# titisda/graph-python

Hardware: AMD Instinct MI355X
Metric: GTEPS (masked mxv/vxm level-BFS, R-MAT s22) (higher is better)
Workload: dtype bool; 1 GPU; level-BFS q<!v.S,replace> = q any.pair A (GxB_ANY_PAIR_BOOL; GrB_vxm, GrB_mxv on A^T shards for N>1), R-MAT scale 22, edge factor 16, 16 roots; n=4194304, nnz=65243197, parallelism=single GPU

## Files before the change

### graph-python_amd/csrc/gb_context.cpp

```cpp
#include <algorithm>
#include <chrono>
#include <cstdio>
#include <cstdio>
#include <cstdlib>
#include <atomic>
#include <map>
#include <mutex>
#include <unordered_map>
#include <vector>

#include <cstring>
#include <dlfcn.h>

#include "gb_internal.h"

namespace {
bool g_init = false;
int g_device = 0;
hipStream_t g_own_stream = nullptr;
hipStream_t g_user_stream = nullptr;
bool g_user_stream_set = false;
std::mutex g_knob_mu;
std::map<std::string, int64_t> g_knobs;
std::atomic<bool> g_any_knob{false};
// ... 314 lines not shown
    g_live[p] = cls;
    return p;
}

void gb_free(void *p) {
    if (!p) return;
    std::lock_guard<std::mutex> lk(g_mem_mu);
    auto it = g_live.find(p);
    if (it == g_live.end()) {
        (void)hipFreeAsync(p, gb_stream());
        return;
    }
    size_t cls = it->second;
    g_live.erase(it);
    if (cls > kCacheLimit) {
        (void)hipFreeAsync(p, gb_stream());
        return;
    }
    while (g_cached_bytes + cls > kCacheLimit && !g_lru.empty()) evict_oldest_locked();
    const uint64_t seq = ++g_free_seq;
    g_cache[cls].push_back(gb_cached{p, seq});
    g_lru.emplace(seq, std::make_pair(p, cls));
    g_cached_bytes += cls;
}

void gb_memset(void *p, int v, size_t bytes) {
    if (bytes) GB_HIP(hipMemsetAsync(p, v, bytes, gb_stream()));
}
void gb_copy_d2d(void *dst, const void *src, size_t bytes) {
    if (bytes) GB_HIP(hipMemcpyAsync(dst, src, bytes, hipMemcpyDeviceToDevice, gb_stream()));
}
void gb_copy_h2d(void *dst, const void *src, size_t bytes) {
    if (bytes) GB_HIP(hipMemcpyAsync(dst, src, bytes, hipMemcpyHostToDevice, gb_stream()));
}
void gb_copy_d2h(void *dst, const void *src, size_t bytes) {
    if (bytes && bytes <= kPinned) {
        std::lock_guard<std::mutex> lk(g_pin_mu);
        if (!g_pinned) GB_HIP(hipHostMalloc(&g_pinned, kPinned, hipHostMallocDefault));
        GB_HIP(hipMemcpyAsync(g_pinned, src, bytes, hipMemcpyDeviceToHost, gb_stream()));
        gb_sync();
        memcpy(dst, g_pinned, bytes);
        return;
    }
    if (bytes) GB_HIP(hipMemcpyAsync(dst, src, bytes, hipMemcpyDeviceToHost, gb_stream()));
    gb_sync();
}
int64_t gb_read_i64(const int64_t *dptr) {
    int64_t v = 0;
    gb_copy_d2h(&v, dptr, sizeof(v));
    return v;
}

int64_t gb_iso_ts_dump();

static const char *k_type_names[] = {"BOOL", "INT8", "UINT8", "INT16", "UINT16", "INT32",
                                     "UINT32", "INT64", "UINT64", "FP32", "FP64"};
static const size_t k_type_sizes[] = {1, 1, 1, 2, 2, 4, 4, 8, 8, 4, 8};
const char *gb_type_name(int code) { return k_type_names[code]; }
size_t gb_type_size(int code) { return k_type_sizes[code]; }
GrB_Type gb_type_of(int code) {
    switch (code) {
    case GBAMD_T_BOOL: return GrB_BOOL;
    case GBAMD_T_INT8: return GrB_INT8;
    case GBAMD_T_UINT8: return GrB_UINT8;
    case GBAMD_T_INT16: return GrB_INT16;
    case GBAMD_T_UINT16: return GrB_UINT16;
    case GBAMD_T_INT32: return GrB_INT32;
    case GBAMD_T_UINT32: return GrB_UINT32;
    case GBAMD_T_INT64: return GrB_INT64;
    case GBAMD_T_UINT64: return GrB_UINT64;
    case GBAMD_T_FP32: return GrB_FP32;
    default: return GrB_FP64;
    }
}

gb_desc gb_read_desc(const GrB_Descriptor d) {
    gb_desc r;
    if (!d) return r;
    GB_REQUIRE(d->magic == GB_MAGIC, GrB_UNINITIALIZED_OBJECT, "invalid descriptor");
    r.replace = d->outp == GrB_REPLACE;
    r.comp = (d->mask & GrB_COMP) != 0;
    r.structure = (d->mask & GrB_STRUCTURE) != 0;
    r.tran0 = d->inp0 == GrB_TRAN;
    r.tran1 = d->inp1 == GrB_TRAN;
    return r;
}

extern "C" {

static int32_t g_mode = GrB_NONBLOCKING;

GrB_Info GrB_init(GrB_Mode mode) {
    return gb_api(nullptr, [&] {
        GB_REQUIRE(!g_init, GrB_INVALID_VALUE, "GrB_init called twice");
        GB_REQUIRE(mode == GrB_BLOCKING || mode == GrB_NONBLOCKING, GrB_INVALID_VALUE, "invalid mode");
        gb_do_init();
        g_mode = mode;
    });
}

GrB_Info GxB_Global_Option_get_INT32(GxB_Option_Field field, int32_t *value) {
    if (!value) return GrB_NULL_POINTER;
    if (field != GxB_MODE) return GrB_INVALID_VALUE;
    *value = g_mode;
    return GrB_SUCCESS;
}

GrB_Info GrB_finalize(void) {
    return gb_api(nullptr, [&] {
        if (!g_init) return;
        GB_HIP(hipDeviceSynchronize());
    });
}

GrB_Info GrB_getVersion(unsigned int *version, unsigned int *subversion) {
    if (!version || !subversion) return GrB_NULL_POINTER;
    *version = GRB_VERSION;
    *subversion = GRB_SUBVERSION;
    return GrB_SUCCESS;
}

GrB_Info GxB_Context_set_stream(void *hip_stream) {
    return gb_api(nullptr, [&] {
        gb_require_init();
        GB_HIP(hipStreamSynchronize(gb_stream()));
        g_user_stream = (hipStream_t)hip_stream;
        g_user_stream_set = hip_stream != nullptr;
    });
}

GrB_Info GxB_Context_get_stream(void **hip_stream) {
    if (!hip_stream) return GrB_NULL_POINTER;
    return gb_api(nullptr, [&] { *hip_stream = (void *)gb_stream(); });
}

GrB_Info GxB_Context_set_device(int device) {
    if (g_init) return GrB_INVALID_VALUE;
    g_device = device;
    return GrB_SUCCESS;
}

GrB_Info GxB_Global_set_int(const char *key, int64_t value) {
    if (!key) return GrB_NULL_POINTER;
    std::lock_guard<std::mutex> lk(g_knob_mu);
    g_knobs[key] = value;
    if (!strcmp(key, "grid_cap")) g_grid_cap.store(value > 0 ? value : 0, std::memory_order_relaxed);
    g_any_knob.store(true, std::memory_order_release);
    return GrB_SUCCESS;
}

GrB_Info GxB_Global_get_int(const char *key, int64_t *value) {
    if (!key || !value) return GrB_NULL_POINTER;
    if (gb_deferred_stat(key, value)) return GrB_SUCCESS;
    if (!strcmp(key, "stat_spmv_host_push")) {
        *value = g_stat_host_push.load(std::memory_order_relaxed);
        return GrB_SUCCESS;
    }
    if (!strcmp(key, "stat_nvals_copy")) {
        *value = g_stat_nvals_copy.load(std::memory_order_relaxed);
        return GrB_SUCCESS;
    }
    if (!strcmp(key, "iso_ts_dump")) {
        return gb_api(nullptr, [&] { *value = gb_iso_ts_dump(); });
    }
    {
        bool mine = false;
        const GrB_Info info = gb_api(nullptr, [&] { mine = gb_sort_stat(key, value) || gb_selectk_stat(key, value); });
        if (mine || info != GrB_SUCCESS) return info;
    }
    if (!strncmp(key, "stat_", 5)) {
        const GrB_Info info = gb_api(nullptr, [&] { gb_union_stat_refresh(key); });
        if (info != GrB_SUCCESS) return info;
        if (!gb_stat_get(key + 5, value)) *value = 0;
        return GrB_SUCCESS;
    }
    *value = gb_knob(key);
    return GrB_SUCCESS;
}

GrB_Info GxB_builtin_lookup(void **handle, int *kind, const char *name) {
    if (!handle || !kind || !name) return GrB_NULL_POINTER;
    static std::map<std::string, const GB_builtin_entry *> *idx = nullptr;
    static std::mutex mu;
    {
        std::lock_guard<std::mutex> lk(mu);
        if (!idx) {
            idx = new std::map<std::string, const GB_builtin_entry *>();
            for (const GB_builtin_entry *e = GB_builtin_registry; e->name; e++) (*idx)[e->name] = e;
        }
    }
    auto it = idx->find(name);
    if (it == idx->end()) return GrB_INVALID_VALUE;
    *handle = it->second->obj;
    *kind = it->second->kind;
    return GrB_SUCCESS;
}

GrB_Info GxB_name(const char **name, const void *obj) {
    if (!name || !obj) return GrB_NULL_POINTER;
    for (const GB_builtin_entry *e = GB_builtin_registry; e->name; e++) {
        if (e->obj == obj) {
            *name = e->name;
            return GrB_SUCCESS;
        }
    }
    return GrB_INVALID_VALUE;
// ... 88 lines not shown
```

### graph-python_amd/csrc/gb_internal.h

```cpp
#pragma once
#include <atomic>
#include <utility>
#include <hip/hip_runtime.h>

#include <cstdint>
#include <cstring>
#include <stdexcept>
#include <string>
#include <vector>

#include "../../include/gbamd_codes.h"
#include "gb_state.h"
#include "../../include/graphblas_amd.h"

#define GB_MAGIC 0x6d614d424731ULL
#define GB_FREED 0x646565724642ULL

struct GB_Type_opaque {
    uint64_t magic;
    int code;
    size_t size;
    const char *name;
};
struct GB_BinaryOp_opaque {
// ... 231 lines not shown
struct gb_scratch {
    void *ptrs[32];
    int n = 0;
    template <class T>
    T *get(size_t count) {
        T *p = gb_malloc_n<T>(count ? count : 1);
        ptrs[n++] = p;
        return p;
    }
    ~gb_scratch() {
        for (int i = 0; i < n; i++) gb_free(ptrs[i]);
    }
};

GB_Obj *gb_obj_check(const void *p, bool allow_null = false);
GB_Obj *gb_obj_check_raw(const void *p, bool allow_null = false);
void gb_cw_to_csr(GB_Obj *A);
void gb_cw_release(GB_Obj *A);
void gb_cw_materialize(GB_Obj *A);
GB_Obj *gb_new_object(int kind, GrB_Type type, int64_t nrows, int64_t ncols);
extern "C" void gb_vec_recount(GB_Obj *v);
void gb_obj_free_storage(GB_Obj *A);
void gb_drop_transpose(GB_Obj *A);
int64_t gb_nvals(GB_Obj *A);
inline int64_t gb_words(int64_t n) { return (n + 63) >> 6; }
inline bool gb_is_bitmap(const GB_Obj *A) { return A->kind != GB_KIND_MATRIX; }

void gb_cast_array(void *dst, int dst_code, const void *src, int src_code, int64_t n);

struct gb_csr_view {
    int64_t nrows = 0, ncols = 0, nvals = 0;
    const int64_t *rowptr = nullptr;
    const int32_t *colidx = nullptr;
    const void *vals = nullptr;
    bool iso = false;
    int tcode = 0;
    const int32_t *hubs = nullptr;
    int64_t nhubs = 0, hub_H = 0;
    const uint64_t *nonempty = nullptr;
    const uint32_t *ne_rank = nullptr;
    const int32_t *phead = nullptr;
    const uint32_t *pdeg = nullptr;
    int64_t maxdeg = -1;
    const int32_t *lchunks = nullptr;
    int64_t nlchunks = -1;
    const void *nvx = nullptr;
    int nvk = 0;
    const int32_t *hcolidx = nullptr;
    const int32_t *hcols = nullptr;
    int64_t nhot = 0;
    gb_scratch own;
};
void gb_get_csr(gb_csr_view &v, GB_Obj *A);
void gb_view_hubs(gb_csr_view &v, GB_Obj *A, int orient, int64_t H);
void gb_view_nonempty(gb_csr_view &v, GB_Obj *A, int orient);
void gb_view_pullfirst(gb_csr_view &v, GB_Obj *A, int orient, const int64_t *other_rowptr, int64_t other_n);
void gb_view_long_rows(gb_csr_view &v, GB_Obj *A, int orient);
void gb_view_narrow(gb_csr_view &v, GB_Obj *A, int orient);
void gb_view_hot(gb_csr_view &v, GB_Obj *A, int orient);
void gb_get_csc(gb_csr_view &v, GB_Obj *A);
const int64_t *gb_csc_perm(GB_Obj *A);
const void *gb_view_vals_as(gb_csr_view &v, int code, gb_scratch &s);

struct gb_bitmap_view {
    int64_t n = 0;
    const uint64_t *bits = nullptr;
    const void *vals = nullptr;
    bool iso = false;
    int tcode = 0;
    const int64_t *count = nullptr;
    const long long *mf_hint = nullptr;
    const void *hint_key = nullptr;
    bool full = false;
    int64_t h_nvals = -1;
    gb_scratch own;
};
void gb_get_bitmap(gb_bitmap_view &v, GB_Obj *A);
const void *gb_bitmap_vals_as(gb_bitmap_view &v, int code, gb_scratch &s);

void gb_install_csr(GB_Obj *C, int64_t nrows, int64_t ncols, int64_t nvals, int64_t *rowptr,
                    int32_t *colidx, void *vals, bool iso);
void gb_install_bitmap(GB_Obj *C, int64_t n, uint64_t *bits, void *dense, bool iso,
                       int64_t *d_nvals );

void gb_bitmap_count(const uint64_t *bits, int64_t n, int64_t *d_count);
void gb_bitmap_to_csr(const uint64_t *bits, const void *dense, bool iso, int64_t n, size_t tsize,
                      int64_t **rowptr, int32_t **colidx, void **vals, int64_t *nvals);
void gb_csr_col_to_bitmap(const gb_csr_view &v, size_t tsize, uint64_t **bits, void **dense,
                          int64_t **d_nvals);

void gb_build(GB_Obj *C, const GrB_Index *I, const GrB_Index *J, const void *X, int xcode, bool x_iso,
              int64_t n, GrB_BinaryOp dup);
void gb_extract_tuples(GB_Obj *A, GrB_Index *I, GrB_Index *J, void *X, int xcode, GrB_Index *nvals);

void *gb_expand_iso(const void *one_value, size_t tsize, int64_t n);

void gb_transpose_csr(int64_t nrows, int64_t ncols, int64_t nvals, const int64_t *rowptr,
                      const int32_t *colidx, const void *vals, size_t tsize, bool iso,
                      int64_t **trowptr, int32_t **tcolidx, void **tvals, int64_t **tperm = nullptr);

struct gb_index_list {
    bool all = false;
    int64_t n = 0;
    std::vector<int64_t> idx;
};
void gb_expand_indices(gb_index_list &L, const GrB_Index *I, GrB_Index ni, int64_t n);
// ... 188 lines not shown
```

### graph-python_amd/csrc/gb_mxv.hip

```cpp
#include "gb_dispatch.cuh"
#include "gb_internal.h"

#define SPMV_TILE 256

template <class SR, class X, class Z, bool FLIP>
__global__ __launch_bounds__(SPMV_BLOCK) void k_spmv_pull(
    SR sr, int64_t nrows, const int64_t *__restrict__ rowptr, const int32_t *__restrict__ colidx,
    const X *__restrict__ avals, bool a_iso, const uint64_t *__restrict__ ubits,
    const X *__restrict__ uvals, bool u_iso, const uint64_t *__restrict__ mbits, bool mcomp, int lg,
    uint64_t *__restrict__ tbits, Z *__restrict__ tvals, unsigned long long *__restrict__ tcount,
    unsigned long long *__restrict__ gst) {
    __shared__ unsigned long long words[SPMV_TILE / 64];
    const int G = 1 << lg;
    const int gid = threadIdx.x >> lg;
    const int gl = threadIdx.x & (G - 1);
    const int ngroups = SPMV_BLOCK >> lg;
    const int lane = threadIdx.x & 63;
    const unsigned long long gmask = (G == 64) ? ~0ULL : (((1ULL << G) - 1) << (lane & ~(G - 1)));
    const int64_t nwords = (nrows + 63) >> 6;
    const bool rv = SR::reads_values && avals && uvals;
    X a0 = X(), u0 = X();
    if (rv) {
        if (a_iso) a0 = avals[0];
        if (u_iso) u0 = uvals[0];
// ... 384 lines not shown
        const unsigned long long fmask = __ballot(hit);
        if (hit) tvals[r] = acc[lane];
        if (lane == 0) {
            tbits[w] = fmask;
            cnt += __popcll(fmask);
        }
        fl[lane] = 0;
        gb_wave_sync();
    }
    long long tot;
    if (gb_grid_sum(cnt, gst, &tot)) *tcount = (unsigned long long)tot;
}

template <class X>
__global__ void k_hot_gather(const X *__restrict__ uvals, const int32_t *__restrict__ hcols, int64_t nh,
                             X *__restrict__ uhot) {
    for (int64_t h = blockIdx.x * (int64_t)blockDim.x + threadIdx.x; h < nh; h += (int64_t)gridDim.x * blockDim.x)
        uhot[h] = uvals[hcols[h]];
}

template <class SR, class Z>
__global__ void k_spmv_fold(SR sr, const int32_t *__restrict__ chunks, int64_t nchunks, const Z *__restrict__ cpart,
                            const int8_t *__restrict__ cfound, uint64_t *__restrict__ tbits, Z *__restrict__ tvals,
                            unsigned long long *__restrict__ tcount, unsigned long long *__restrict__ gst) {
    long long cnt = 0;
    for (int64_t c = blockIdx.x * (int64_t)blockDim.x + threadIdx.x; c < nchunks;
         c += (int64_t)gridDim.x * blockDim.x) {
        if (chunks[2 * c + 1] != 0) continue;
        const int64_t r = chunks[2 * c];
        bool f = false;
        Z z = Z();
        for (int64_t h = c; h < nchunks && chunks[2 * h] == r; h++) {
            if (!cfound[h]) continue;
            z = f ? sr.add(z, cpart[h]) : cpart[h];
            f = true;
        }
        if (f) {
            tvals[r] = z;
            atomicOr((unsigned long long *)&tbits[r >> 6], 1ULL << (r & 63));
            cnt++;
        }
    }
    gb_grid_add(cnt, tcount, gst);
}

__global__ void k_hub_count(const int64_t *__restrict__ rowptr, int64_t n, int64_t thresh, int64_t H,
                            int64_t *__restrict__ cnt) {
    for (int64_t r = blockIdx.x * (int64_t)blockDim.x + threadIdx.x; r < n; r += (int64_t)gridDim.x * blockDim.x) {
        const int64_t d = rowptr[r + 1] - rowptr[r];
        cnt[r] = d > thresh ? (d + H - 1) / H : 0;
    }
}
__global__ void k_hub_fill(const int64_t *__restrict__ cnt, const int64_t *__restrict__ off, int64_t n,
                           int32_t *__restrict__ tab) {
    for (int64_t r = blockIdx.x * (int64_t)blockDim.x + threadIdx.x; r < n; r += (int64_t)gridDim.x * blockDim.x) {
        const int64_t c = cnt[r], o = off[r];
        for (int64_t i = 0; i < c; i++) {
            tab[2 * (o + i)] = (int32_t)r;
            tab[2 * (o + i) + 1] = (int32_t)i;
        }
    }
}

static int32_t *gb_build_chunk_table(const gb_csr_view &v, int64_t thresh, int64_t H, int64_t *total_out) {
    const int64_t n = v.nrows;
    gb_scratch s;
    int64_t *cnt = s.get<int64_t>(n + 1);
    int64_t *off = s.get<int64_t>(n + 1);
    const unsigned g = gb_grid(n, 256, 8192);
    hipLaunchKernelGGL(k_hub_count, dim3(g), dim3(256), 0, gb_stream(), v.rowptr, n, thresh, H, cnt);
    GB_LAUNCH_CHECK();
    gb_exclusive_scan_i64(cnt, off, n);
    const int64_t total = gb_read_i64(off + n);
    int32_t *tab = gb_malloc_n<int32_t>(2 * total + 2);
    hipLaunchKernelGGL(k_hub_fill, dim3(g), dim3(256), 0, gb_stream(), cnt, off, n, tab);
    GB_LAUNCH_CHECK();
    *total_out = total;
    return tab;
}

__global__ void k_row_maxlen(const int64_t *__restrict__ rowptr, int64_t n, unsigned long long *__restrict__ mx) {
    unsigned long long m = 0;
    for (int64_t r = blockIdx.x * (int64_t)blockDim.x + threadIdx.x; r < n; r += (int64_t)gridDim.x * blockDim.x) {
        const unsigned long long d = (unsigned long long)(rowptr[r + 1] - rowptr[r]);
        m = d > m ? d : m;
    }
    for (int off = 32; off > 0; off >>= 1) {
        const unsigned long long o = __shfl_xor(m, off, 64);
        m = o > m ? o : m;
    }
    if ((threadIdx.x & 63) == 0 && m) atomicMax(mx, m);
}

void gb_view_hubs(gb_csr_view &v, GB_Obj *A, int orient, int64_t H) {
    if (A->kind != GB_KIND_MATRIX) return;
    gb_orient_cache &c = A->oc[orient];
    if (!c.hub_tab || c.hub_H != H) {
        gb_stat_add("hub_tables_built", 1);
        gb_free(c.hub_tab);
        c.hub_tab = gb_build_chunk_table(v, H, H, &c.hub_n);
        c.hub_H = H;
        gb_scratch s;
        unsigned long long *mx = s.get<unsigned long long>(1);
        gb_memset(mx, 0, sizeof(unsigned long long));
        const unsigned g = gb_grid(v.nrows, 256, 2048);
        hipLaunchKernelGGL(k_row_maxlen, dim3(g), dim3(256), 0, gb_stream(), v.rowptr, v.nrows, mx);
        GB_LAUNCH_CHECK();
        unsigned long long h = 0;
        gb_copy_d2h(&h, mx, sizeof(h));
        c.maxdeg = (int64_t)h;
    }
    v.hubs = c.hub_tab;
    v.nhubs = c.hub_n;
    v.hub_H = H;
    v.maxdeg = c.maxdeg;
}

void gb_view_long_rows(gb_csr_view &v, GB_Obj *A, int orient) {
    if (A->kind != GB_KIND_MATRIX) return;
    gb_orient_cache &c = A->oc[orient];
    if (!c.long_tab) {
        gb_stat_add("long_tables_built", 1);
        c.long_tab = gb_build_chunk_table(v, SPMV_LONG, SPMV_CH, &c.long_n);
    }
    v.lchunks = c.long_tab;
    v.nlchunks = c.long_n;
}

__global__ void k_rows_nonempty(const int64_t *__restrict__ rowptr, int64_t n, uint64_t *__restrict__ ne,
                                int32_t *__restrict__ pc) {
    const int lane = threadIdx.x & 63;
    const int64_t nw = (n + 63) >> 6;
    for (int64_t w = (blockIdx.x * (int64_t)blockDim.x + threadIdx.x) >> 6; w < nw;
         w += ((int64_t)gridDim.x * blockDim.x) >> 6) {
        const int64_t r = (w << 6) + lane;
        const unsigned long long b = __ballot(r < n && rowptr[r + 1] > rowptr[r]);
        if (lane == 0) {
            ne[w] = b;
            pc[w] = __popcll(b);
        }
    }
}

__global__ void k_narrow_u32(const int64_t *__restrict__ in, uint32_t *__restrict__ out, int64_t n) {
    GB_GRID_LOOP(i, n)
        out[i] = (uint32_t)in[i];
}

void gb_view_nonempty(gb_csr_view &v, GB_Obj *A, int orient) {
    if (A->kind != GB_KIND_MATRIX) return;
    gb_orient_cache &c = A->oc[orient];
    if (!c.rows_ne) {
        gb_stat_add("nonempty_built", 1);
// ... 193 lines not shown
```

### graph-python_amd/csrc/gb_spmv_iso.hip

```cpp
#include <mutex>

#include "gb_dispatch.cuh"
#include "gb_internal.h"

enum { ST_PUSH = 0 };
#define PULL_U 4

struct gb_dir_rule {
    const int64_t *mask_count;
    const int64_t *extra_count;
    bool mcomp;
    int64_t n_out, nnz, alpha;
    int force_push;
};

__device__ __forceinline__ bool gb_dir_decide(long long mf, const gb_dir_rule &rule) {
    int64_t open = rule.n_out;
    if (rule.mask_count) {
        int64_t mc = *rule.mask_count;
        if (rule.extra_count) mc += *rule.extra_count;
        if (mc > rule.n_out) mc = rule.n_out;
        open = rule.mcomp ? (rule.n_out - mc) : mc;
    }
    const double avg = rule.n_out ? (double)rule.nnz / (double)rule.n_out : 0.0;
    return rule.force_push || ((double)mf * (double)rule.alpha < (double)open * avg);
}

__global__ __launch_bounds__(SPMV_BLOCK) void k_dir_prep(
    const uint64_t *__restrict__ ubits, int64_t nwords_u, const int64_t *__restrict__ prow,
    unsigned long long *__restrict__ gst, unsigned long long *__restrict__ dst,
    uint64_t *__restrict__ tbits, int64_t nwords_out, unsigned long long *__restrict__ tcount, gb_dir_rule rule) {
    const int lane = threadIdx.x & 63;
    const int64_t wave = (blockIdx.x * (int64_t)blockDim.x + threadIdx.x) >> 6;
    const int64_t nwaves = ((int64_t)gridDim.x * blockDim.x) >> 6;
    long long mf = 0;
    for (int64_t base = wave * 16; base < nwords_u; base += nwaves * 16) {
        const int64_t wl = base + (lane & 15);
        const uint64_t mine = wl < nwords_u ? ubits[wl] : 0;
        unsigned long long nz = __ballot(mine != 0) & 0xFFFFULL;
        while (nz) {
            int64_t deg[4];
#pragma unroll
            for (int u = 0; u < 4; u++) {
                deg[u] = 0;
                if (nz) {
                    const int l = __ffsll(nz) - 1;
                    nz &= nz - 1;
                    const uint64_t word = __shfl(mine, l, 64);
                    if ((word >> lane) & 1ULL) {
                        const int64_t k = ((base + l) << 6) + lane;
                        deg[u] = prow[k + 1] - prow[k];
                    }
                }
            }
#pragma unroll
            for (int u = 0; u < 4; u++) mf += deg[u];
        }
    }
    const int64_t tid = blockIdx.x * (int64_t)blockDim.x + threadIdx.x;
    for (int64_t w = tid; w < nwords_out; w += (int64_t)gridDim.x * blockDim.x) tbits[w] = 0;
    if (tid == 0) *tcount = 0;
    long long total;
    if (gb_grid_sum(mf, gst, &total)) dst[ST_PUSH] = gb_dir_decide(total, rule) ? 1ULL : 0ULL;
}

__device__ __forceinline__ long long gb_push_targets(const int32_t (&j)[4], bool (&ok)[4],
                                                     const uint64_t *__restrict__ mbits, bool mcomp,
                                                     unsigned long long *__restrict__ tbits,
                                                     const int64_t *__restrict__ hprow, long long &mfn,
                                                     const uint64_t *__restrict__ qbits, bool serial = false,
                                                     int64_t qroot = -1) {
    unsigned long long cur[4];
    if (serial) {
        if (mbits) {
#pragma unroll
            for (int u = 0; u < 4; u++)
                if (ok[u]) ok[u] = (gb_bit(mbits, j[u]) || (qbits && gb_bit(qbits, j[u]))) != mcomp;
        }
#pragma unroll
        for (int u = 0; u < 4; u++) cur[u] = ok[u] ? tbits[j[u] >> 6] : ~0ULL;
    } else {
        uint64_t mw[4], qw[4];
#pragma unroll
        for (int u = 0; u < 4; u++) {
            mw[u] = qw[u] = 0;
            cur[u] = ~0ULL;
            if (ok[u]) {
                if (mbits) mw[u] = mbits[j[u] >> 6];
                if (mbits && qbits) qw[u] = qbits[j[u] >> 6];
                cur[u] = tbits[j[u] >> 6];
            }
        }
        if (mbits) {
#pragma unroll
            for (int u = 0; u < 4; u++)
                if (ok[u]) ok[u] = (((((mw[u] | qw[u]) >> (j[u] & 63)) & 1ULL) != 0) || j[u] == qroot) != mcomp;
        }
    }
    long long added = 0;
#pragma unroll
    for (int u = 0; u < 4; u++) {
        const unsigned long long m = 1ULL << (j[u] & 63);
        if (ok[u] && !(cur[u] & m)) {
            const unsigned long long old = atomicOr(&tbits[j[u] >> 6], m);
            if (!(old & m)) {
                added++;
                if (hprow) mfn += hprow[j[u] + 1] - hprow[j[u]];
            }
        }
    }
    return added;
}

#define WL_MAX 256
struct gb_wlist {
    int64_t p[WL_MAX];
    int32_t rem[WL_MAX];
    int32_t pref[WL_MAX];
    int16_t id[WL_MAX];
    int8_t hit[WL_MAX];
    unsigned long long hitw[PULL_U];
};

__device__ __forceinline__ int gb_wlist_round(gb_wlist &L, int n, int cap, int lane) {
    int v[4], sum = 0;
#pragma unroll
    for (int t = 0; t < 4; t++) {
        const int i = lane * 4 + t;
        v[t] = 0;
        if (i < n) {
            v[t] = L.rem[i] < cap ? L.rem[i] : cap;
            L.hit[i] = 0;
        }
        sum += v[t];
    }
    int incl = sum;
    for (int off = 1; off < 64; off <<= 1) {
        const int y = __shfl_up(incl, off, 64);
        if (lane >= off) incl += y;
    }
    int run = incl - sum;
#pragma unroll
    for (int t = 0; t < 4; t++) {
        const int i = lane * 4 + t;
        run += v[t];
        if (i < n) L.pref[i] = run;
    }
    gb_wave_sync();
    return __shfl(incl, 63, 64);
}

__device__ __forceinline__ int gb_wlist_start(const gb_wlist &L, int i) { return i ? L.pref[i - 1] : 0; }

__device__ __forceinline__ int gb_wlist_find(const gb_wlist &L, int n, int e) {
    int lo = 0;
#pragma unroll
    for (int st = WL_MAX / 2; st > 0; st >>= 1)
        if (lo + st <= n && L.pref[lo + st - 1] <= e) lo += st;
    return lo;
}

__device__ __forceinline__ int gb_wlist_survivors(gb_wlist &L, int n, int lane, unsigned long long lt) {
// ... 13 lines not shown
            alive = !hit && nr > 0;
        }
        if (hit) atomicOr(&L.hitw[id >> 6], 1ULL << (id & 63));
        const unsigned long long ab = __ballot(alive);
        gb_wave_sync();
        if (alive) {
            const int j = m + __popcll(ab & lt);
            L.p[j] = np;
            L.rem[j] = nr;
            L.id[j] = id;
        }
        m += __popcll(ab);
        gb_wave_sync();
    }
    return m;
}

struct gb_asg_dev {
    uint64_t *bits;
    void *vals;
    int size;
    unsigned long long x;
};
__device__ __forceinline__ void gb_store_sized(void *base, int64_t i, int size, unsigned long long x) {
    switch (size) {
    case 1: ((uint8_t *)base)[i] = (uint8_t)x; break;
    case 2: ((uint16_t *)base)[i] = (uint16_t)x; break;
    case 4: ((uint32_t *)base)[i] = (uint32_t)x; break;
    default: ((unsigned long long *)base)[i] = x; break;
    }
}
__device__ __forceinline__ long long gb_asg_words(const gb_asg_dev &g, int64_t w0, int64_t nwords, uint64_t qw,
                                                 int lane, const uint64_t *cpre = nullptr) {
    long long added = 0;
    const int64_t wl = w0 + (lane & 3);
    if (lane < 4 && wl < nwords && qw) {
        const uint64_t c = cpre ? *cpre : g.bits[wl], nwd = c | qw;
        if (nwd != c) g.bits[wl] = nwd;
        added = (long long)__popcll(nwd) - (long long)__popcll(c);
    }
#pragma unroll
    for (int u = 0; u < 4; u++) {
        const uint64_t word = __shfl(qw, u, 64);
        if ((word >> lane) & 1ULL) gb_store_sized(g.vals, ((w0 + u) << 6) + lane, g.size, g.x);
    }
    return added;
}

__device__ __forceinline__ long long gb_push_phase(int64_t nwords_u, const uint64_t *__restrict__ ubits,
                                                  const int64_t *__restrict__ prow, const int32_t *__restrict__ pcol,
                                                  const int32_t *__restrict__ hubs, int64_t nhubs, int64_t H,
                                                  const uint64_t *__restrict__ mbits, bool mcomp,
                                                  unsigned long long *__restrict__ tbits, gb_wlist &L,
                                                  const int64_t *__restrict__ hprow, long long &mfn,
                                                  const uint64_t *__restrict__ qbits, const gb_asg_dev &g,
                                                  long long &adelta, bool serial = false, bool prefetch = true,
                                                  bool defer = false) {
    const int lane = threadIdx.x & 63;
    const int64_t wave = (blockIdx.x * (int64_t)blockDim.x + threadIdx.x) >> 6;
    const int64_t nwaves = ((int64_t)gridDim.x * blockDim.x) >> 6;
    const unsigned long long lt = (1ULL << lane) - 1;
    long long added = 0;
    uint64_t pre = 0;
    {
        const int64_t wl = wave * 4 + (int64_t)(lane >> 2) * nwaves * 4 + (lane & 3);
        if (wl < nwords_u) pre = ubits[wl];
    }
    for (int64_t base = wave; base < nhubs; base += nwaves * 16) {
        const int64_t h = base + (int64_t)lane * nwaves;
        int k = 0, cc = 0;
        bool act = false;
        if (lane < 16 && h < nhubs) {
            k = hubs[2 * h];
            cc = hubs[2 * h + 1];
            act = gb_bit(ubits, k);
        }
        unsigned long long b = __ballot(act);
        while (b) {
            const int l = __ffsll(b) - 1;
            b &= b - 1;
            const int64_t kk = __shfl(k, l, 64);
            const int64_t c = __shfl(cc, l, 64);
            const int64_t p0 = prow[kk] + c * H, pe = prow[kk + 1];
            const int64_t p1 = (p0 + H < pe) ? p0 + H : pe;
            for (int64_t p = p0 + lane; p < p1; p += 256) {
                int32_t j[4];
                bool ok[4];
#pragma unroll
                for (int u = 0; u < 4; u++) {
                    ok[u] = p + 64 * u < p1;
                    j[u] = ok[u] ? pcol[p + 64 * u] : 0;
                }
                added += gb_push_targets(j, ok, mbits, mcomp, tbits, hprow, mfn, qbits, serial);
            }
        }
    }
    int n = 0;
    auto flush = [&]() {
        gb_wave_sync();
        const int total = gb_wlist_round(L, n, 1 << 30, lane);
        for (int e0 = 0; e0 < total; e0 += 256) {
            int32_t j[4];
            bool ok[4];
#pragma unroll
            for (int u = 0; u < 4; u++) {
                const int e = e0 + lane + 64 * u;
                ok[u] = e < total;
                j[u] = 0;
                if (ok[u]) {
                    const int s = gb_wlist_find(L, n, e);
                    j[u] = pcol[L.p[s] + (e - gb_wlist_start(L, s))];
                }
            }
            added += gb_push_targets(j, ok, mbits, mcomp, tbits, hprow, mfn, qbits, serial);
        }
        gb_wave_sync();
        n = 0;
    };
    int step = 0;
    for (int64_t w0 = wave * 4; w0 < nwords_u; w0 += nwaves * 4, step++) {
        const int64_t wl = w0 + (lane & 3);
        uint64_t mine;
        if (prefetch && step < 16) {
            mine = __shfl(pre, (step << 2) | (lane & 3), 64);
        } else {
            mine = wl < nwords_u ? ubits[wl] : 0;
        }
        if (!__ballot(mine != 0)) continue;
        if (qbits) adelta += gb_asg_words(g, w0, nwords_u, mine, lane);
        int64_t p0[4], d[4];
#pragma unroll
        for (int u = 0; u < 4; u++) {
            const uint64_t word = __shfl(mine, u, 64);
            p0[u] = d[u] = 0;
            if ((word >> lane) & 1ULL) {
                const int64_t k = ((w0 + u) << 6) + lane;
                p0[u] = prow[k];
                d[u] = prow[k + 1] - p0[u];
            }
        }
        unsigned long long bb[4];
        int add = 0;
#pragma unroll
        for (int u = 0; u < 4; u++) {
            bb[u] = __ballot(d[u] > 0 && d[u] <= H);
            add += __popcll(bb[u]);
        }
        if (!add) continue;
        if (n + add > WL_MAX) flush();
#pragma unroll
        for (int u = 0; u < 4; u++) {
            if ((bb[u] >> lane) & 1ULL) {
                const int i = n + __popcll(bb[u] & lt);
                L.p[i] = p0[u];
                L.rem[i] = (int32_t)d[u];
            }
            n += __popcll(bb[u]);
        }
        if (!defer) flush();
    }
    if (n) flush();
    return added;
}

__device__ __forceinline__ long long gb_push_root(int64_t root, const int64_t *__restrict__ prow,
                                                 const int32_t *__restrict__ pcol,
                                                 const uint64_t *__restrict__ mbits, bool mcomp,
                                                 unsigned long long *__restrict__ tbits,
                                                 const int64_t *__restrict__ hprow, long long &mfn, bool stamp,
                                                 const gb_asg_dev &g, long long &adelta) {
    const int lane = threadIdx.x & 63;
    const int64_t wave = (blockIdx.x * (int64_t)blockDim.x + threadIdx.x) >> 6;
    const int64_t nwaves = ((int64_t)gridDim.x * blockDim.x) >> 6;
    if (stamp && blockIdx.x == 0 && threadIdx.x == 0) {
        const unsigned long long m = 1ULL << (root & 63);
        const unsigned long long old = atomicOr((unsigned long long *)&g.bits[root >> 6], m);
        gb_store_sized(g.vals, root, g.size, g.x);
        if (!(old & m)) adelta += 1;
    }
    const int64_t p0 = prow[root], p1 = prow[root + 1];
    long long added = 0;
    for (int64_t p = p0 + wave * 256 + lane; p < p1; p += nwaves * 256) {
        int32_t j[4];
        bool ok[4];
#pragma unroll
        for (int u = 0; u < 4; u++) {
            ok[u] = p + 64 * u < p1;
            j[u] = ok[u] ? pcol[p + 64 * u] : 0;
        }
        added += gb_push_targets(j, ok, mbits, mcomp, tbits, hprow, mfn, nullptr, false, stamp ? root : -1);
    }
    return added;
}

__device__ __forceinline__ uint32_t gb_ne_rank(uint32_t prefix, uint64_t rw, int bit) {
    return prefix + (uint32_t)__popcll(rw & ((1ULL << bit) - 1));
}
__device__ __forceinline__ uint64_t gb_readlane64(uint64_t x, int l) {
    const uint32_t lo = (uint32_t)__builtin_amdgcn_readlane((int)(uint32_t)x, l);
    const uint32_t hi = (uint32_t)__builtin_amdgcn_readlane((int)(uint32_t)(x >> 32), l);
    return ((uint64_t)hi << 32) | lo;
}

__device__ __forceinline__ void gb_pull_probe_heads(const int4 (&hv)[PULL_U], const uint64_t *__restrict__ ubits,
                                                    bool (&found)[PULL_U]) {
    const uint32_t *ub32 = reinterpret_cast<const uint32_t *>(ubits);
    uint32_t w1[PULL_U];
#pragma unroll
    for (int u = 0; u < PULL_U; u++) {
        w1[u] = 0;
        if (hv[u].x >= 0) w1[u] = ub32[hv[u].x >> 5];
    }
#pragma unroll
    for (int u = 0; u < PULL_U; u++) found[u] = hv[u].x >= 0 && ((w1[u] >> (hv[u].x & 31)) & 1u);
    uint32_t wy[PULL_U], wz[PULL_U], ww[PULL_U];
#pragma unroll
    for (int u = 0; u < PULL_U; u++) {
        wy[u] = wz[u] = ww[u] = 0;
        if (!found[u]) {
            if (hv[u].y >= 0) wy[u] = ub32[hv[u].y >> 5];
            if (hv[u].z >= 0) wz[u] = ub32[hv[u].z >> 5];
            if (hv[u].w >= 0) ww[u] = ub32[hv[u].w >> 5];
        }
    }
#pragma unroll
    for (int u = 0; u < PULL_U; u++)
        found[u] = found[u] || (hv[u].y >= 0 && ((wy[u] >> (hv[u].y & 31)) & 1u)) ||
                   (hv[u].z >= 0 && ((wz[u] >> (hv[u].z & 31)) & 1u)) ||
                   (hv[u].w >= 0 && ((ww[u] >> (hv[u].w & 31)) & 1u));
}

__device__ __forceinline__ void gb_wlist_walk_pull(gb_wlist &L, int n, int cap0, const int32_t *__restrict__ colidx,
                                                   const uint64_t *__restrict__ ubits) {
    const int lane = threadIdx.x & 63;
    const unsigned long long lt = (1ULL << lane) - 1;
    int cap = cap0;
    while (n) {
        gb_wave_sync();
        const int total = gb_wlist_round(L, n, cap, lane);
        for (int e0 = 0; e0 < total; e0 += 256) {
            int k[4], s[4];
            bool ok[4];
#pragma unroll
// ... 479 lines not shown
__global__ __launch_bounds__(SPMV_BLOCK) void k_iso_work(
    int64_t nrows, const int64_t *__restrict__ rowptr, const int32_t *__restrict__ colidx,
    int64_t nwords_u, const uint64_t *__restrict__ ubits, const int64_t *__restrict__ prow,
    const int32_t *__restrict__ pcol, const int32_t *__restrict__ hubs, int64_t nhubs, int64_t H,
    const uint64_t *__restrict__ mbits, bool mcomp, uint64_t *__restrict__ tbits,
    unsigned long long *__restrict__ tcount, unsigned long long *__restrict__ gst, gb_iso_args a) {
    __shared__ gb_wlist lists[WAVES_PER_BLOCK];
    gb_wlist &L = lists[threadIdx.x >> 6];
    __shared__ gb_wpack packs[WAVES_PER_BLOCK];
    if (a.ts && blockIdx.x == 0 && threadIdx.x == 0) iso_ts_mark(a, 0);
    if (a.dbg & 8) return;
    bool push = false;
    if (a.host_dir == 1) {
        push = true;
    } else if (a.mf_hint) {
        long long mf = 0;
        for (int i = 0; i < GB_HINT_PARTS; i++) mf += a.mf_hint[i];
        push = gb_dir_decide(mf, a.rule);
    }
    else if (a.dst) push = a.dst[ST_PUSH] != 0;
    if (a.spare && !(a.dbg & 32)) {
        for (int64_t w = blockIdx.x * (int64_t)blockDim.x + threadIdx.x; w < a.spare_words;
             w += (int64_t)gridDim.x * blockDim.x)
            a.spare[w] = 0;
    }
    for (int j = 0; j < ((a.dbg & 32) ? 0 : a.nzb); j++)
        for (int64_t w = blockIdx.x * (int64_t)blockDim.x + threadIdx.x; w < a.zb_words;
             w += (int64_t)gridDim.x * blockDim.x)
            a.zb[j][w] = 0;
    if (blockIdx.x == 0)
        for (int j = 0; j < a.nzc; j++)
            for (int w = threadIdx.x; w < 2 + GB_HINT_PARTS; w += blockDim.x) a.zc[j][w] = 0;
    if (a.packed && a.iso_out && blockIdx.x == 0 && threadIdx.x == 0)
        gb_iso_eval(a.mul, a.xcode, a.zcode, a.flip, a.a0, a.u0, a.iso_out);
    if (a.u_exit && *a.u_exit == 0) {
        if (!a.out_zeroed)
            for (int64_t w = blockIdx.x * (int64_t)blockDim.x + threadIdx.x; w < ((nrows + 63) >> 6);
                 w += (int64_t)gridDim.x * blockDim.x)
                tbits[w] = 0;
        if (blockIdx.x == 0) {
            if (a.mf_out)
                for (int i = threadIdx.x; i < GB_HINT_PARTS; i += blockDim.x) a.mf_out[i] = 0;
            if (threadIdx.x == 0) {
                *tcount = 0ULL;
                if (!a.packed && a.iso_out) gb_iso_eval(a.mul, a.xcode, a.zcode, a.flip, a.a0, a.u0, a.iso_out);
                iso_publish(a, 0);
            }
        }
        return;
    }
    const uint64_t *qbits = nullptr;
    if (a.asg.bits && (!a.asg_qiso || gb_dyn_nonzero(a.asg_qiso, a.asg_qiso_code))) qbits = ubits;
    long long mfn = 0, cnt = 0, adelta = 0;
    if (a.dbg & 4)
        ;
    else if (a.root >= 0)
        cnt = gb_push_root(a.root, prow, pcol, mbits, mcomp, (unsigned long long *)tbits, a.hprow, mfn,
                           a.asg.bits != nullptr, a.asg, adelta);
    else if (push)
        cnt = gb_push_phase(nwords_u, ubits, prow, pcol, hubs, nhubs, H, mbits, mcomp,
                            (unsigned long long *)tbits, L, a.hprow, mfn, qbits, a.asg, adelta, (a.dbg & 128) != 0,
                            (a.dbg & 512) == 0, (a.pack & 2) != 0);
    else {
        const int32_t *ph =
            (a.phead && a.rows_nonempty && a.ne_rank && (!a.hprow || a.pdeg)) ? a.phead : nullptr;
        if ((a.pack & 1) && ph && a.p1_steps == 0 && !(a.dbg & (16 | 32 | 128)))
            cnt = gb_pull_iso_packed(nrows, rowptr, colidx, ubits, mbits, mcomp, tbits, L, packs[threadIdx.x >> 6],
                                     a.hprow, mfn, a.cap0, a.rows_nonempty, qbits, a.asg, adelta, ph, a.pdeg, a.ne_rank);
        else
            cnt = gb_pull_iso_phase(nrows, rowptr, colidx, ubits, mbits, mcomp, tbits, L, a.hprow, mfn, a.p1_steps,
                                    a.cap0, a.rows_nonempty, qbits, a.asg, adelta, a.dbg, ph, a.pdeg, a.ne_rank);
    }
    if (a.dbg & 64) return;
    if (a.packed) {
        iso_finish_packed(cnt, mfn, adelta, tcount, gst, a);
        return;
    }
    long long tot;
    if (gb_grid_sum(cnt, gst, &tot)) {
        *tcount = (unsigned long long)tot;
        if (a.iso_out) gb_iso_eval(a.mul, a.xcode, a.zcode, a.flip, a.a0, a.u0, a.iso_out);
        iso_publish(a, tot);
    }
    if (a.mf_out && !(a.dbg & 2)) {
        long long m;
        if (gb_grid_sum(mfn, gst + GB_GRID2_OFFSET, &m)) {
            a.mf_out[0] = m;
            for (int i = 1; i < GB_HINT_PARTS; i++) a.mf_out[i] = 0;
        }
    }
    if (a.asg.bits) gb_grid_add(adelta, a.asg_count, gst + GB_GRID3_OFFSET);
}

static std::mutex g_dir_mu;
static unsigned long long *g_iso_ts = nullptr;
static unsigned long long *iso_ts_buffer() {
    static const bool on = getenv("GRAPHBLAS_AMD_ISO_TS") != nullptr;
    if (!on) return nullptr;
    if (!g_iso_ts) {
        GB_HIP(hipMalloc((void **)&g_iso_ts, (2 + 2 * (size_t)ISO_TS_PAIRS) * sizeof(unsigned long long)));
        GB_HIP(hipMemset(g_iso_ts, 0, (2 + 2 * (size_t)ISO_TS_PAIRS) * sizeof(unsigned long long)));
        GB_HIP(hipDeviceSynchronize());
    }
    return g_iso_ts;
}
int64_t gb_iso_ts_dump() {
    const char *path = getenv("GRAPHBLAS_AMD_ISO_TS");
    if (!path || !g_iso_ts) return 0;
    GB_HIP(hipStreamSynchronize(gb_stream()));
    unsigned long long c[2];
    GB_HIP(hipMemcpy(c, g_iso_ts, sizeof(c), hipMemcpyDeviceToHost));
    const size_t k = std::min<unsigned long long>(std::min(c[0], c[1]), ISO_TS_PAIRS);
    std::vector<unsigned long long> buf(2 + 2 * k);
    GB_HIP(hipMemcpy(buf.data(), g_iso_ts, buf.size() * sizeof(unsigned long long), hipMemcpyDeviceToHost));
    FILE *f = fopen(path, "wb");
// ... 214 lines not shown
```

Baseline: 346.1 GTEPS.

## Restructure push phase with packed hub pieces, 32-bit bit atomics and overlapped loads

Builds an extended hub table holding 16-byte per-piece records (row, length, start position) and a u32 row-length array, so the push kernel fetches one record per hub chunk instead of recomputing bounds from rowptr. The length array also replaces the 64-bit hprow difference used for the direction-switch work estimate. Visited-bit checks and atomicOr now operate on 32-bit words, with loads and atomics batched across an 8-wide unroll for hub chunks. The first frontier-word row loads are interleaved with the hub-entry fetch to overlap latency. It also adds a per-launch device counter for push launches, which costs one extra atomic per launch. The work estimate now comes from this matrix's own row lengths, which may not equal the degrees hprow used to supply.

```diff
diff --git a/graph-python_amd/csrc/gb_context.cpp b/graph-python_amd/csrc/gb_context.cpp
--- a/graph-python_amd/csrc/gb_context.cpp
+++ b/graph-python_amd/csrc/gb_context.cpp
@@ -390,6 +390,7 @@
 }
 
 int64_t gb_iso_ts_dump();
+int64_t gb_iso_push_launches();
 
 static const char *k_type_names[] = {"BOOL", "INT8", "UINT8", "INT16", "UINT16", "INT32",
                                      "UINT32", "INT64", "UINT64", "FP32", "FP64"};
@@ -490,6 +491,9 @@
 GrB_Info GxB_Global_get_int(const char *key, int64_t *value) {
     if (!key || !value) return GrB_NULL_POINTER;
     if (gb_deferred_stat(key, value)) return GrB_SUCCESS;
+    if (!strcmp(key, "stat_iso_push_launches")) {
+        return gb_api(nullptr, [&] { *value = gb_iso_push_launches(); });
+    }
     if (!strcmp(key, "stat_spmv_host_push")) {
         *value = g_stat_host_push.load(std::memory_order_relaxed);
         return GrB_SUCCESS;
diff --git a/graph-python_amd/csrc/gb_internal.h b/graph-python_amd/csrc/gb_internal.h
--- a/graph-python_amd/csrc/gb_internal.h
+++ b/graph-python_amd/csrc/gb_internal.h
@@ -307,6 +307,24 @@
     gb_scratch own;
 };
 void gb_get_csr(gb_csr_view &v, GB_Obj *A);
+struct gb_hub_piece {
+    int32_t row;
+    int32_t len;
+    int64_t pos;
+};
+static_assert(sizeof(gb_hub_piece) == 16, "one 16-byte load per piece");
+struct gb_hub_sections {
+    const gb_hub_piece *piece = nullptr;
+    const uint32_t *rowlen = nullptr;
+};
+__host__ __device__ inline int64_t gb_hub_prefix_ints(int64_t nhubs) { return (2 * nhubs + 2 + 3) & ~(int64_t)3; }
+__host__ __device__ inline gb_hub_sections gb_hub_sections_of(const int32_t *tab, int64_t nhubs) {
+    gb_hub_sections s;
+    s.piece = reinterpret_cast<const gb_hub_piece *>(tab + gb_hub_prefix_ints(nhubs));
+    s.rowlen = reinterpret_cast<const uint32_t *>(s.piece + nhubs);
+    return s;
+}
+inline int64_t gb_hub_table_ints(int64_t nhubs, int64_t nrows) { return gb_hub_prefix_ints(nhubs) + 4 * nhubs + nrows; }
 void gb_view_hubs(gb_csr_view &v, GB_Obj *A, int orient, int64_t H);
 void gb_view_nonempty(gb_csr_view &v, GB_Obj *A, int orient);
 void gb_view_pullfirst(gb_csr_view &v, GB_Obj *A, int orient, const int64_t *other_rowptr, int64_t other_n);
diff --git a/graph-python_amd/csrc/gb_mxv.hip b/graph-python_amd/csrc/gb_mxv.hip
--- a/graph-python_amd/csrc/gb_mxv.hip
+++ b/graph-python_amd/csrc/gb_mxv.hip
@@ -460,17 +460,27 @@
     }
 }
 __global__ void k_hub_fill(const int64_t *__restrict__ cnt, const int64_t *__restrict__ off, int64_t n,
-                           int32_t *__restrict__ tab) {
+                           int32_t *__restrict__ tab, const int64_t *__restrict__ rowptr, int64_t H,
+                           gb_hub_piece *__restrict__ rec) {
     for (int64_t r = blockIdx.x * (int64_t)blockDim.x + threadIdx.x; r < n; r += (int64_t)gridDim.x * blockDim.x) {
         const int64_t c = cnt[r], o = off[r];
         for (int64_t i = 0; i < c; i++) {
             tab[2 * (o + i)] = (int32_t)r;
             tab[2 * (o + i) + 1] = (int32_t)i;
-        }
-    }
-}
-
-static int32_t *gb_build_chunk_table(const gb_csr_view &v, int64_t thresh, int64_t H, int64_t *total_out) {
+            if (rec) {
+                const int64_t p0 = rowptr[r] + i * H, left = rowptr[r + 1] - p0;
+                rec[o + i] = gb_hub_piece{(int32_t)r, (int32_t)(left < H ? left : H), p0};
+            }
+        }
+    }
+}
+__global__ void k_row_len_u32(const int64_t *__restrict__ rowptr, int64_t n, uint32_t *__restrict__ out) {
+    GB_GRID_LOOP(r, n)
+        out[r] = (uint32_t)(rowptr[r + 1] - rowptr[r]);
+}
+
+static int32_t *gb_build_chunk_table(const gb_csr_view &v, int64_t thresh, int64_t H, int64_t *total_out,
+                                     bool sections = false) {
     const int64_t n = v.nrows;
     gb_scratch s;
     int64_t *cnt = s.get<int64_t>(n + 1);
@@ -480,9 +490,16 @@
     GB_LAUNCH_CHECK();
     gb_exclusive_scan_i64(cnt, off, n);
     const int64_t total = gb_read_i64(off + n);
-    int32_t *tab = gb_malloc_n<int32_t>(2 * total + 2);
-    hipLaunchKernelGGL(k_hub_fill, dim3(g), dim3(256), 0, gb_stream(), cnt, off, n, tab);
+    int32_t *tab = gb_malloc_n<int32_t>(sections ? gb_hub_table_ints(total, n) : 2 * total + 2);
+    const gb_hub_sections sec = sections ? gb_hub_sections_of(tab, total) : gb_hub_sections{};
+    hipLaunchKernelGGL(k_hub_fill, dim3(g), dim3(256), 0, gb_stream(), cnt, off, n, tab, v.rowptr, H,
+                       const_cast<gb_hub_piece *>(sec.piece));
     GB_LAUNCH_CHECK();
+    if (sections) {
+        hipLaunchKernelGGL(k_row_len_u32, dim3(g), dim3(256), 0, gb_stream(), v.rowptr, n,
+                           const_cast<uint32_t *>(sec.rowlen));
+        GB_LAUNCH_CHECK();
+    }
     *total_out = total;
     return tab;
 }
@@ -506,7 +523,7 @@
     if (!c.hub_tab || c.hub_H != H) {
         gb_stat_add("hub_tables_built", 1);
         gb_free(c.hub_tab);
-        c.hub_tab = gb_build_chunk_table(v, H, H, &c.hub_n);
+        c.hub_tab = gb_build_chunk_table(v, H, H, &c.hub_n, true);
         c.hub_H = H;
         gb_scratch s;
         unsigned long long *mx = s.get<unsigned long long>(1);
diff --git a/graph-python_amd/csrc/gb_spmv_iso.hip b/graph-python_amd/csrc/gb_spmv_iso.hip
--- a/graph-python_amd/csrc/gb_spmv_iso.hip
+++ b/graph-python_amd/csrc/gb_spmv_iso.hip
@@ -3,7 +3,13 @@
 #include "gb_dispatch.cuh"
 #include "gb_internal.h"
 
-enum { ST_PUSH = 0 };
+enum { ST_PUSH = 0, ST_PUSHES = 1 };
+int64_t gb_iso_push_launches() {
+    unsigned long long c = 0;
+    GB_HIP(hipStreamSynchronize(gb_stream()));
+    GB_HIP(hipMemcpy(&c, gb_device_state() + GB_DIR_STATE_OFFSET + ST_PUSHES, sizeof(c), hipMemcpyDeviceToHost));
+    return (int64_t)c;
+}
 #define PULL_U 4
 
 struct gb_dir_rule {
@@ -64,50 +70,65 @@
     if (gb_grid_sum(mf, gst, &total)) dst[ST_PUSH] = gb_dir_decide(total, rule) ? 1ULL : 0ULL;
 }
 
-__device__ __forceinline__ long long gb_push_targets(const int32_t (&j)[4], bool (&ok)[4],
+template <int W>
+__device__ __forceinline__ long long gb_push_targets(const int32_t (&j)[W], bool (&ok)[W],
                                                      const uint64_t *__restrict__ mbits, bool mcomp,
                                                      unsigned long long *__restrict__ tbits,
-                                                     const int64_t *__restrict__ hprow, long long &mfn,
+                                                     const uint32_t *__restrict__ hlen, long long &mfn,
                                                      const uint64_t *__restrict__ qbits, bool serial = false,
                                                      int64_t qroot = -1) {
-    unsigned long long cur[4];
+    uint32_t cur[W];
+    const uint32_t *t32 = reinterpret_cast<const uint32_t *>(tbits);
     if (serial) {
         if (mbits) {
 #pragma unroll
-            for (int u = 0; u < 4; u++)
+            for (int u = 0; u < W; u++)
                 if (ok[u]) ok[u] = (gb_bit(mbits, j[u]) || (qbits && gb_bit(qbits, j[u]))) != mcomp;
         }
 #pragma unroll
-        for (int u = 0; u < 4; u++) cur[u] = ok[u] ? tbits[j[u] >> 6] : ~0ULL;
+        for (int u = 0; u < W; u++) cur[u] = ok[u] ? t32[j[u] >> 5] : ~0u;
     } else {
-        uint64_t mw[4], qw[4];
-#pragma unroll
-        for (int u = 0; u < 4; u++) {
+        const uint32_t *m32 = reinterpret_cast<const uint32_t *>(mbits);
+        const uint32_t *q32 = reinterpret_cast<const uint32_t *>(qbits);
+        uint32_t mw[W], qw[W];
+#pragma unroll
+        for (int u = 0; u < W; u++) {
             mw[u] = qw[u] = 0;
-            cur[u] = ~0ULL;
+            cur[u] = ~0u;
             if (ok[u]) {
-                if (mbits) mw[u] = mbits[j[u] >> 6];
-                if (mbits && qbits) qw[u] = qbits[j[u] >> 6];
-                cur[u] = tbits[j[u] >> 6];
+                if (mbits) mw[u] = m32[j[u] >> 5];
+                if (mbits && qbits) qw[u] = q32[j[u] >> 5];
+                cur[u] = t32[j[u] >> 5];
             }
         }
         if (mbits) {
 #pragma unroll
-            for (int u = 0; u < 4; u++)
-                if (ok[u]) ok[u] = (((((mw[u] | qw[u]) >> (j[u] & 63)) & 1ULL) != 0) || j[u] == qroot) != mcomp;
-        }
-    }
+            for (int u = 0; u < W; u++)
+                if (ok[u]) ok[u] = (((((mw[u] | qw[u]) >> (j[u] & 31)) & 1u) != 0) || j[u] == qroot) != mcomp;
+        }
+    }
+    unsigned int *t32w = reinterpret_cast<unsigned int *>(tbits);
+    uint32_t old[W];
+    bool won[W];
+#pragma unroll
+    for (int u = 0; u < W; u++) {
+        old[u] = cur[u];
+        won[u] = ok[u] && !((cur[u] >> (j[u] & 31)) & 1u);
+    }
+#pragma unroll
+    for (int u = 0; u < W; u++)
+        if (won[u]) old[u] = atomicOr(&t32w[j[u] >> 5], 1u << (j[u] & 31));
+#pragma unroll
+    for (int u = 0; u < W; u++) won[u] = won[u] && !((old[u] >> (j[u] & 31)) & 1u);
     long long added = 0;
 #pragma unroll
-    for (int u = 0; u < 4; u++) {
-        const unsigned long long m = 1ULL << (j[u] & 63);
-        if (ok[u] && !(cur[u] & m)) {
-            const unsigned long long old = atomicOr(&tbits[j[u] >> 6], m);
-            if (!(old & m)) {
-                added++;
-                if (hprow) mfn += hprow[j[u] + 1] - hprow[j[u]];
-            }
-        }
+    for (int u = 0; u < W; u++) added += won[u] ? 1 : 0;
+    if (hlen) {
+        uint32_t dl[W];
+#pragma unroll
+        for (int u = 0; u < W; u++) dl[u] = hlen[won[u] ? j[u] : 0];
+#pragma unroll
+        for (int u = 0; u < W; u++) mfn += won[u] ? dl[u] : 0u;
     }
     return added;
 }
@@ -227,7 +248,7 @@
                                                   const int32_t *__restrict__ hubs, int64_t nhubs, int64_t H,
                                                   const uint64_t *__restrict__ mbits, bool mcomp,
                                                   unsigned long long *__restrict__ tbits, gb_wlist &L,
-                                                  const int64_t *__restrict__ hprow, long long &mfn,
+                                                  const uint32_t *__restrict__ hlen, long long &mfn,
                                                   const uint64_t *__restrict__ qbits, const gb_asg_dev &g,
                                                   long long &adelta, bool serial = false, bool prefetch = true,
                                                   bool defer = false) {
@@ -235,41 +256,45 @@
     const int64_t wave = (blockIdx.x * (int64_t)blockDim.x + threadIdx.x) >> 6;
     const int64_t nwaves = ((int64_t)gridDim.x * blockDim.x) >> 6;
     const unsigned long long lt = (1ULL << lane) - 1;
+    const gb_hub_sections sec = gb_hub_sections_of(hubs, nhubs);
     long long added = 0;
     uint64_t pre = 0;
     {
         const int64_t wl = wave * 4 + (int64_t)(lane >> 2) * nwaves * 4 + (lane & 3);
         if (wl < nwords_u) pre = ubits[wl];
     }
-    for (int64_t base = wave; base < nhubs; base += nwaves * 16) {
+    int hk = -1, hl = 0;
+    int64_t hp = 0;
+    uint64_t hw;
+    auto hub_entry = [&](int64_t base) {
         const int64_t h = base + (int64_t)lane * nwaves;
-        int k = 0, cc = 0;
-        bool act = false;
+        hk = -1;
         if (lane < 16 && h < nhubs) {
-            k = hubs[2 * h];
-            cc = hubs[2 * h + 1];
-            act = gb_bit(ubits, k);
-        }
-        unsigned long long b = __ballot(act);
-        while (b) {
-            const int l = __ffsll(b) - 1;
-            b &= b - 1;
-            const int64_t kk = __shfl(k, l, 64);
-            const int64_t c = __shfl(cc, l, 64);
-            const int64_t p0 = prow[kk] + c * H, pe = prow[kk + 1];
-            const int64_t p1 = (p0 + H < pe) ? p0 + H : pe;
-            for (int64_t p = p0 + lane; p < p1; p += 256) {
-                int32_t j[4];
-                bool ok[4];
-#pragma unroll
-                for (int u = 0; u < 4; u++) {
-                    ok[u] = p + 64 * u < p1;
-                    j[u] = ok[u] ? pcol[p + 64 * u] : 0;
-                }
-                added += gb_push_targets(j, ok, mbits, mcomp, tbits, hprow, mfn, qbits, serial);
-            }
-        }
-    }
+            const gb_hub_piece pc = sec.piece[h];
+            hk = pc.row;
+            hl = pc.len;
+            hp = pc.pos;
+        }
+    };
+    if (wave < nhubs) hub_entry(wave);
+    auto rows_load = [&](int64_t w0, uint64_t mine, int64_t (&p0)[4], int64_t (&d)[4], uint64_t &cw) {
+        const int64_t wl = w0 + (lane & 3);
+        cw = 0;
+        if (qbits && lane < 4 && wl < nwords_u && mine) cw = g.bits[wl];
+        int64_t p1[4];
+#pragma unroll
+        for (int u = 0; u < 4; u++) {
+            const uint64_t word = __shfl(mine, u, 64);
+            p0[u] = p1[u] = 0;
+            if ((word >> lane) & 1ULL) {
+                const int64_t k = ((w0 + u) << 6) + lane;
+                p0[u] = prow[k];
+                p1[u] = prow[k + 1];
+            }
+        }
+#pragma unroll
+        for (int u = 0; u < 4; u++) d[u] = p1[u] - p0[u];
+    };
     int n = 0;
     auto flush = [&]() {
         gb_wave_sync();
@@ -287,13 +312,77 @@
                     j[u] = pcol[L.p[s] + (e - gb_wlist_start(L, s))];
                 }
             }
-            added += gb_push_targets(j, ok, mbits, mcomp, tbits, hprow, mfn, qbits, serial);
+            added += gb_push_targets<4>(j, ok, mbits, mcomp, tbits, hlen, mfn, qbits, serial);
         }
         gb_wave_sync();
         n = 0;
     };
+    auto rows_add = [&](int64_t w0, uint64_t mine, const int64_t (&p0)[4], const int64_t (&d)[4], uint64_t cw) {
+        if (qbits) adelta += gb_asg_words(g, w0, nwords_u, mine, lane, &cw);
+        unsigned long long bb[4];
+        int add = 0;
+#pragma unroll
+        for (int u = 0; u < 4; u++) {
+            bb[u] = __ballot(d[u] > 0 && d[u] <= H);
+            add += __popcll(bb[u]);
+        }
+        if (!add) return;
+        if (n + add > WL_MAX) flush();
+#pragma unroll
+        for (int u = 0; u < 4; u++) {
+            if ((bb[u] >> lane) & 1ULL) {
+                const int i = n + __popcll(bb[u] & lt);
+                L.p[i] = p0[u];
+                L.rem[i] = (int32_t)d[u];
+            }
+            n += __popcll(bb[u]);
+        }
+    };
     int step = 0;
-    for (int64_t w0 = wave * 4; w0 < nwords_u; w0 += nwaves * 4, step++) {
+    int64_t w0 = wave * 4;
+    bool act;
+    {
+        const bool first = prefetch && w0 < nwords_u;
+        const uint64_t mine = first ? __shfl(pre, lane & 3, 64) : 0;
+        int64_t p0[4], d[4];
+        uint64_t cw;
+        const bool any = __ballot(mine != 0) != 0;
+        __builtin_amdgcn_sched_barrier(0);
+        hw = ubits[(hk >= 0 ? hk : 0) >> 6];
+        if (any) rows_load(w0, mine, p0, d, cw);
+        act = hk >= 0 && ((hw >> (hk & 63)) & 1ULL);
+        if (any) rows_add(w0, mine, p0, d, cw);
+        if (first) {
+            step = 1;
+            w0 += nwaves * 4;
+        }
+    }
+    for (int64_t base = wave; base < nhubs;) {
+        unsigned long long b = __ballot(act);
+        while (b) {
+            const int l = __ffsll(b) - 1;
+            b &= b - 1;
+            const int64_t pp = __shfl(hp, l, 64);
+            const int ln = __shfl(hl, l, 64);
+            for (int e0 = lane; e0 < ln; e0 += 512) {
+                int32_t j[8];
+                bool ok[8];
+#pragma unroll
+                for (int u = 0; u < 8; u++) {
+                    ok[u] = e0 + 64 * u < ln;
+                    j[u] = ok[u] ? pcol[pp + e0 + 64 * u] : 0;
+                }
+                added += gb_push_targets<8>(j, ok, mbits, mcomp, tbits, hlen, mfn, qbits, serial);
+            }
+        }
+        base += nwaves * 16;
+        if (base >= nhubs) break;
+        hub_entry(base);
+        hw = ubits[(hk >= 0 ? hk : 0) >> 6];
+        act = hk >= 0 && ((hw >> (hk & 63)) & 1ULL);
+    }
+    if (n && !defer) flush();
+    for (; w0 < nwords_u; w0 += nwaves * 4, step++) {
         const int64_t wl = w0 + (lane & 3);
         uint64_t mine;
         if (prefetch && step < 16) {
@@ -302,37 +391,11 @@
             mine = wl < nwords_u ? ubits[wl] : 0;
         }
         if (!__ballot(mine != 0)) continue;
-        if (qbits) adelta += gb_asg_words(g, w0, nwords_u, mine, lane);
         int64_t p0[4], d[4];
-#pragma unroll
-        for (int u = 0; u < 4; u++) {
-            const uint64_t word = __shfl(mine, u, 64);
-            p0[u] = d[u] = 0;
-            if ((word >> lane) & 1ULL) {
-                const int64_t k = ((w0 + u) << 6) + lane;
-                p0[u] = prow[k];
-                d[u] = prow[k + 1] - p0[u];
-            }
-        }
-        unsigned long long bb[4];
-        int add = 0;
-#pragma unroll
-        for (int u = 0; u < 4; u++) {
-            bb[u] = __ballot(d[u] > 0 && d[u] <= H);
-            add += __popcll(bb[u]);
-        }
-        if (!add) continue;
-        if (n + add > WL_MAX) flush();
-#pragma unroll
-        for (int u = 0; u < 4; u++) {
-            if ((bb[u] >> lane) & 1ULL) {
-                const int i = n + __popcll(bb[u] & lt);
-                L.p[i] = p0[u];
-                L.rem[i] = (int32_t)d[u];
-            }
-            n += __popcll(bb[u]);
-        }
-        if (!defer) flush();
+        uint64_t cw;
+        rows_load(w0, mine, p0, d, cw);
+        rows_add(w0, mine, p0, d, cw);
+        if (n && !defer) flush();
     }
     if (n) flush();
     return added;
@@ -342,8 +405,8 @@
                                                  const int32_t *__restrict__ pcol,
                                                  const uint64_t *__restrict__ mbits, bool mcomp,
                                                  unsigned long long *__restrict__ tbits,
-                                                 const int64_t *__restrict__ hprow, long long &mfn, bool stamp,
-                                                 const gb_asg_dev &g, long long &adelta) {
+                                                 const uint32_t *__restrict__ hlen, long long &mfn,
+                                                 bool stamp, const gb_asg_dev &g, long long &adelta) {
     const int lane = threadIdx.x & 63;
     const int64_t wave = (blockIdx.x * (int64_t)blockDim.x + threadIdx.x) >> 6;
     const int64_t nwaves = ((int64_t)gridDim.x * blockDim.x) >> 6;
@@ -363,7 +426,7 @@
             ok[u] = p + 64 * u < p1;
             j[u] = ok[u] ? pcol[p + 64 * u] : 0;
         }
-        added += gb_push_targets(j, ok, mbits, mcomp, tbits, hprow, mfn, nullptr, false, stamp ? root : -1);
+        added += gb_push_targets<4>(j, ok, mbits, mcomp, tbits, hlen, mfn, nullptr, false, stamp ? root : -1);
     }
     return added;
 }
@@ -949,15 +1012,18 @@
     const uint64_t *qbits = nullptr;
     if (a.asg.bits && (!a.asg_qiso || gb_dyn_nonzero(a.asg_qiso, a.asg_qiso_code))) qbits = ubits;
     long long mfn = 0, cnt = 0, adelta = 0;
+    if ((a.root >= 0 || push) && blockIdx.x == 0 && threadIdx.x == 0)
+        atomicAdd(gst + GB_DIR_STATE_OFFSET + ST_PUSHES, 1ULL);
+    const uint32_t *hlen = (a.hprow && hubs) ? gb_hub_sections_of(hubs, nhubs).rowlen : nullptr;
     if (a.dbg & 4)
         ;
     else if (a.root >= 0)
-        cnt = gb_push_root(a.root, prow, pcol, mbits, mcomp, (unsigned long long *)tbits, a.hprow, mfn,
+        cnt = gb_push_root(a.root, prow, pcol, mbits, mcomp, (unsigned long long *)tbits, hlen, mfn,
                            a.asg.bits != nullptr, a.asg, adelta);
     else if (push)
         cnt = gb_push_phase(nwords_u, ubits, prow, pcol, hubs, nhubs, H, mbits, mcomp,
-                            (unsigned long long *)tbits, L, a.hprow, mfn, qbits, a.asg, adelta, (a.dbg & 128) != 0,
-                            (a.dbg & 512) == 0, (a.pack & 2) != 0);
+                            (unsigned long long *)tbits, L, hlen, mfn, qbits, a.asg, adelta,
+                            (a.dbg & 128) != 0, (a.dbg & 512) == 0, (a.pack & 2) != 0);
     else {
         const int32_t *ph =
             (a.phead && a.rows_nonempty && a.ne_rank && (!a.hprow || a.pdeg)) ? a.phead : nullptr;
```

New measurement: 357.2 GTEPS, median of 6. 1.03x the previous value.
